# matthiasverstraete/3d_recognizer

Hardware: AMD Instinct MI355X
Metric: training clouds/sec, N=40960 pts, bs=8, at 1/2/4/8 GPUs; mIoU parity (higher is better)
Workload: dtype f32 storage/accumulate, bf16x3 MFMA in the wide GEMMs

## Files before the change

3d_recognizer_amd/csrc/bn.hip:

```cpp
#include "rl_common.h"

namespace {

__device__ __forceinline__ void slot_sums_wg(const double* __restrict__ stats, int nslots, int C, int c,
                                             double (*red)[2], double& s_out, double& q_out) {
    const int t = threadIdx.x;
    double s = 0.0, q = 0.0;
    const double* base = stats + c;
    for (int i = t; i < nslots; i += 256) {
        s += base[((long)i * 2 + 0) * C];
        q += base[((long)i * 2 + 1) * C];
    }
    s = rl_wave_sum(s);
    q = rl_wave_sum(q);
    if ((t & 63) == 0) { red[t >> 6][0] = s; red[t >> 6][1] = q; }
    __syncthreads();
    s_out = (red[0][0] + red[1][0]) + (red[2][0] + red[3][0]);
    q_out = (red[0][1] + red[1][1]) + (red[2][1] + red[3][1]);
}

__device__ __forceinline__ void slot_sums(const double* __restrict__ stats, int nslots, int C, int c, int lane,
                                          double& s_out, double& q_out) {
    double s0 = 0.0, s1 = 0.0, s2 = 0.0, s3 = 0.0, q0 = 0.0, q1 = 0.0, q2 = 0.0, q3 = 0.0;
    const double* base = stats + c;
// ... 195 lines not shown
                                                                   float* coef0, float* dgamma1, float* dbeta1, float* coef1) {
    __shared__ double red[4][2];
    if (blockIdx.y == 0) bn_bwd_finalize_body(stats0, nslots, count, C, dgamma0, dbeta0, coef0, (int)blockIdx.x, red);
    else bn_bwd_finalize_body(stats1, nslots, count, C, dgamma1, dbeta1, coef1, (int)blockIdx.x, red);
}

constexpr int BNBF_MAX = 8;
struct BnBwdFinBatch {
    rl_bn_bwd_finalize_item it[BNBF_MAX];
};
__global__ __launch_bounds__(256) void bn_bwd_finalize_batch_kernel(const BnBwdFinBatch b) {
    __shared__ double red[4][2];
    const rl_bn_bwd_finalize_item& t = b.it[blockIdx.y];
    if ((int)blockIdx.x >= t.C) return;
    bn_bwd_finalize_body(t.stats, t.nslots, (double)t.count, t.C, t.dgamma, t.dbeta, t.coef, (int)blockIdx.x, red);
}

__global__ __launch_bounds__(256) void bn_bwd_apply_kernel(const BwdParams p) {
    const int C = p.C;
    const int tpr = C < 256 ? C : 256;
    const int rpar = 256 / tpr;
    const int col = threadIdx.x % tpr, rsub = threadIdx.x / tpr;
    if (rsub >= rpar) return;
    const long ntiles = (p.M + p.tile - 1) / p.tile;
    for (long tile = blockIdx.x; tile < ntiles; tile += gridDim.x) {
        const long rend = min(p.M, (tile + 1) * p.tile);
        for (long R = tile * p.tile + rsub; R < rend; R += rpar) {
            const long off = row_off(p, R);
            for (int c = col; c < C; c += 256) {
                const float y = p.Y[off + c];
                const float sc = p.scale ? p.scale[c] : 1.f, sh = p.shift ? p.shift[c] : 0.f;
                float g = p.G[off + c] * rl_act_grad(y * sc + sh, p.act, p.slope);
                if (p.coef) {
                    const float xh = (y - p.mean[c]) * p.invstd[c];
                    g = g - p.coef[c] - xh * p.coef[C + c];
                }
                p.G[off + c] = sc * g;
            }
        }
    }
}

typedef float bnf4 __attribute__((ext_vector_type(4)));
struct BnQuad {
    bnf4 sc, sh, mu, is;
    float neg;
    __device__ __forceinline__ void load(const BwdParams& p, int c, bool want_xhat) {
        sc = p.scale ? *reinterpret_cast<const bnf4*>(p.scale + c) : (bnf4){1.f, 1.f, 1.f, 1.f};
        sh = p.shift ? *reinterpret_cast<const bnf4*>(p.shift + c) : (bnf4){0.f, 0.f, 0.f, 0.f};
        mu = (bnf4){0.f, 0.f, 0.f, 0.f};
        is = mu;
        if (want_xhat) {
            mu = *reinterpret_cast<const bnf4*>(p.mean + c);
            is = *reinterpret_cast<const bnf4*>(p.invstd + c);
        }
        neg = p.act == RL_ACT_RELU ? 0.f : (p.act == RL_ACT_LRELU ? p.slope : 1.f);
    }
    __device__ __forceinline__ bnf4 grad(const bnf4 y, const bnf4 gin) const {
        const bnf4 z = y * sc + sh;
        bnf4 d;
// ... 51 lines not shown
        for (int j = 0; j < 4; ++j) {
            p.stats[((long)blockIdx.x * 2 + 0) * C + c + j] = s[j];
            p.stats[((long)blockIdx.x * 2 + 1) * C + c + j] = s[4 + j];
        }
    }
}

__global__ __launch_bounds__(256) void bn_bwd_apply_vec_kernel(const BwdParams p) {
    const int C = p.C, c4 = C >> 2;
    const int tpr = c4 < 256 ? c4 : 256;
    const int rpar = 256 / tpr;
    const int q = threadIdx.x % tpr, rsub = threadIdx.x / tpr;
    const int c = q * 4;
    const bool full = p.coef != nullptr;
    BnQuad k;
    k.load(p, c, full);
    bnf4 k0 = {0.f, 0.f, 0.f, 0.f}, k1 = k0;
    if (full) {
        k0 = *reinterpret_cast<const bnf4*>(p.coef + c);
        k1 = *reinterpret_cast<const bnf4*>(p.coef + C + c);
    }
    const bnf4 osc = p.scale ? k.sc : (bnf4){1.f, 1.f, 1.f, 1.f};
    auto row = [&](const bnf4 y, const bnf4 gi) {
        bnf4 g = k.grad(y, gi);
        if (full) g = g - k0 - k.xhat(y) * k1;
        return g * osc;
    };
    const long ntiles = (p.M + p.tile - 1) / p.tile;
    for (long tile = blockIdx.x; tile < ntiles; tile += gridDim.x) {
        const long rend = min(p.M, (tile + 1) * p.tile);
        long R = tile * p.tile + rsub;
        for (; R + rpar < rend; R += 2 * rpar) {
            const long o0 = row_off(p, R) + c, o1 = row_off(p, R + rpar) + c;
            const bnf4 y0 = *reinterpret_cast<const bnf4*>(p.Y + o0), g0 = *reinterpret_cast<const bnf4*>(p.G + o0);
            const bnf4 y1 = *reinterpret_cast<const bnf4*>(p.Y + o1), g1 = *reinterpret_cast<const bnf4*>(p.G + o1);
            *reinterpret_cast<bnf4*>(p.G + o0) = row(y0, g0);
            *reinterpret_cast<bnf4*>(p.G + o1) = row(y1, g1);
        }
        if (R < rend) {
            const long o0 = row_off(p, R) + c;
            const bnf4 y0 = *reinterpret_cast<const bnf4*>(p.Y + o0), g0 = *reinterpret_cast<const bnf4*>(p.G + o0);
            *reinterpret_cast<bnf4*>(p.G + o0) = row(y0, g0);
        }
    }
}

struct ResidParams {
    float* G; float* G2; const float* O; float slope; long M; int C;
    const float* Y1; const float* sc1; const float* mu1; const float* is1;
// ... 445 lines not shown
```

3d_recognizer_amd/csrc/gemm.hip:

```cpp
#include "rl_common.h"
#include <stdlib.h>
#include <string.h>

namespace {

typedef float f32x4 __attribute__((ext_vector_type(4)));

constexpr int GM_BM = 128;
constexpr int GM_BK = 16;
constexpr int GM_AS = 20;

struct AOperand {
    const float* A;
    long lda, a_bstride;
    int a_mode;
    RlLazy lazy;
    const float* xyz;
    long xyz_bstride;
    const int32_t* nbr_idx;
    const float* nbr_d2;
    int nbr_k;
    int n;
    int K;
    long M;
// ... 750 lines not shown
template <int KT, int NT>
__global__ __launch_bounds__(256) void swgrad_kernel(const WgradParams p) {
    __shared__ float red[KT * NT * 4 * 64 + NT * 64];
    swgrad_body<KT, NT>(p, (int)blockIdx.x, red);
}

void swgrad_split(long M, int* nsplit, long* rows_per_block) {
    constexpr long rows_wg = 256;
    long want = (M + rows_wg - 1) / rows_wg;
    const long fill = (M + 127) / 128 < 256 ? (M + 127) / 128 : 256;
    if (want < fill) want = fill;
    if (want < 1) want = 1;
    if (want > 1024) want = 1024;
    long rpb = (M + want - 1) / want;
    rpb = ((rpb + 63) / 64) * 64;
    *rows_per_block = rpb;
    *nsplit = (int)((M + rpb - 1) / rpb);
    if (*nsplit < 1) *nsplit = 1;
}

inline bool stream_ok(int N, int K) { return (N <= 64 && K <= 64) || (K <= 16 && N <= 128); }

constexpr int swgrad_body_index(int KT, int NT) { return 4 * (KT >= 4 ? 2 : KT - 1) + (NT >= 8 ? 3 : NT >= 4 ? 2 : NT - 1); }

constexpr int PG_BK = 32;
constexpr int PG_AS = 36;

typedef __attribute__((ext_vector_type(8))) __bf16 bf16x8;
typedef __attribute__((ext_vector_type(4))) __bf16 bf16x4;

template <int NT, bool STATS>
__device__ __forceinline__ void tile_rows_epilogue(const GemmParams& p, const f32x4 (&acc)[NT], long Rb, int col0, int lr, int lq,
                                                   float (&ssum)[NT], float (&ssq)[NT]) {
    constexpr int BN = 16 * NT;
    const int N = p.N;
    const long M = p.a.M;
    const bool to_y = !p.out2 || col0 + BN <= p.split_col;
    const bool to_out2 = p.out2 && !p.out2_index && col0 >= p.split_col;
    if (to_y || to_out2) {
        const bool full = col0 + BN <= N;
        const bool has_bias = p.bias != nullptr;
        const bool accumulate = to_y && p.accumulate;
        float bv[NT];
#pragma unroll
        for (int nb = 0; nb < NT; ++nb) {
            const int c = col0 + nb * 16 + lr;
// ... 2126 lines not shown
extern "C" int rl_wgrad_reduce_batch(const rl_wgrad_reduce_item* items, int count, void* stream) {
    RL_REQUIRE(items != nullptr && count >= 0, RL_ERR_ARGS, "rl_wgrad_reduce_batch: bad arguments");
    hipStream_t st = (hipStream_t)stream;
    for (int base = 0; base < count; base += RB_MAX) {
        ReduceBatch b;
        b.count = count - base < RB_MAX ? count - base : RB_MAX;
        long tiles = 0;
        for (int i = 0; i < b.count; ++i) {
            const rl_wgrad_reduce_item& it = items[base + i];
            RL_REQUIRE(it.slab && it.dW && it.nsplit > 0 && it.N > 0 && it.K > 0, RL_ERR_ARGS,
                       "rl_wgrad_reduce_batch: bad item %d", base + i);
            b.item[i] = it;
            b.first_tile[i] = (int)tiles;
            tiles += rl_cdiv((long)it.N * it.K + it.N, WR_E);
            RL_REQUIRE(tiles < (1l << 30), RL_ERR_ARGS, "rl_wgrad_reduce_batch: too many tiles");
        }
        b.first_tile[b.count] = (int)tiles;
        hipLaunchKernelGGL(wgrad_reduce_batch_kernel, dim3((unsigned)tiles), dim3(256), 0, st, b);
        RL_LAUNCH_CHECK("rl_wgrad_reduce_batch");
    }
    rl_note_kernel("wgrad_reduce_batch_kernel");
    return RL_OK;
}
```

3d_recognizer_amd/csrc/rl_common.h:

```cpp
#pragma once
#include <hip/hip_runtime.h>
#include <stdarg.h>
#include <stdint.h>
#include <stdio.h>

#include "../../include/rl_randlanet.h"

void rl_set_error(const char* fmt, ...);
void rl_note_kernel(const char* name);

#define RL_REQUIRE(cond, code, ...)      \
    do {                                 \
        if (!(cond)) {                   \
            rl_set_error(__VA_ARGS__);   \
            return (code);               \
        }                                \
    } while (0)

#define RL_LAUNCH_CHECK(name)                                                        \
    do {                                                                             \
        hipError_t e_ = hipGetLastError();                                           \
        if (e_ != hipSuccess) {                                                      \
            rl_set_error("%s: launch failed: %s", name, hipGetErrorString(e_));      \
            return RL_ERR_LAUNCH;                                                    \
// ... 17 lines not shown
    const char* e = getenv("RL_ALLOW_FLOAT_ATOMICS");
    return e && e[0] == '1';
}

static inline int rl_row_blocks_host(long rows, int rows_per_tile) {
    long tiles = (rows + rows_per_tile - 1) / rows_per_tile;
    if (tiles < 1) tiles = 1;
    return (int)(tiles < RL_MAX_SLOTS ? tiles : RL_MAX_SLOTS);
}

#define RL_ACT_NONE 0
#define RL_ACT_RELU 1
#define RL_ACT_LRELU 2

__device__ __forceinline__ float rl_act(float z, int act, float slope) {
    if (act == RL_ACT_RELU) return z > 0.f ? z : 0.f;
    if (act == RL_ACT_LRELU) return z > 0.f ? z : z * slope;
    return z;
}
__device__ __forceinline__ float rl_act_grad(float z, int act, float slope) {
    if (act == RL_ACT_RELU) return z > 0.f ? 1.f : 0.f;
    if (act == RL_ACT_LRELU) return z > 0.f ? 1.f : slope;
    return 1.f;
}

struct RlLazy {
    const float* scale;
    const float* shift;
    int act;
    float slope;
};
__device__ __forceinline__ float rl_lazy(const RlLazy& t, float raw, int c) {
    if (t.scale == nullptr) return raw;
    return rl_act(raw * t.scale[c] + t.shift[c], t.act, t.slope);
}

typedef __bf16 rl_bf16x4 __attribute__((ext_vector_type(4)));
template <bool BF>
__device__ __forceinline__ float rl_ldx(const float* p, long i) {
    if constexpr (BF) return (float)reinterpret_cast<const __bf16*>(p)[i];
    else return p[i];
}
template <bool BF>
__device__ __forceinline__ void rl_stx(float* p, long i, float v) {
    if constexpr (BF) reinterpret_cast<__bf16*>(p)[i] = (__bf16)v;
    else p[i] = v;
// ... 55 lines not shown
```

3d_recognizer_amd/randlanet/_engine.py:

```python
from typing import Dict, List, Optional

import torch

from . import _hip as H
from . import _ops as ops
from ._ops import Lazy, Rpe

BN_EPS = 1e-6
BN_MOMENTUM = 0.99
BN_PIVOT = True
BAND_SORT_MIN_POINTS = 4096


class _Tape(list):

    def __init__(self):
        super().__init__()
        self.levels: List[int] = []

    def append(self, rec) -> None:
        super().append(rec)
        self.levels.append(ops.LEVEL)

    def clear(self) -> None:
# ... 458 lines not shown
                ops.scale_mask(G, mask, scale)
                ctx.grads[id(src.raw)] = [G, True]
            else:
                raise AssertionError(kind)
        self._flush_rpe(ctx)
        ops.LEVEL = -1
        ops.wgrad_batch_flush(ctx.wbatch)
        ops.wgrad_flush(ctx.pending)
        ctx.tape.clear()
        ctx.grads.clear()
        ctx.keep.clear()

    def _flush_rpe(self, ctx: Context) -> None:
        if ctx.fin_queue:
            first = ctx.fin_queue.pop(0)
            ops._bn_bwd_finalize(*first, None, also=ctx.fin_queue)
        for fn in ctx.rpe_after:
            fn()
        ctx.rpe_after.clear()

    def _bwd_linear(self, ctx, grads, a, out: Lazy, wname, bname, ks, ns, a_grad):
        G, init = self._gbuf(ctx, out)
        assert init, f"no gradient reached {wname}"
        if out.scale is not None and id(out.raw) not in ctx.bn_done:
            ops.bn_backward(G, out, grads[f"{out.bn}.weight"], grads[f"{out.bn}.bias"], True, sync=self.sync,
                            stats=ctx.bn_pre.pop(id(out.raw), None), also=ctx.fin_queue)
            self._flush_rpe(ctx)
        n_out = out.C
        ops.wgrad(a, G, out.bstride, n_out, grads[wname], ks, ns, grads[bname] if bname else None, pending=ctx.pending,
                  batch=ctx.wbatch)
        halves = getattr(a, "concat", None) if (a_grad and isinstance(a, Lazy)) else None
        if (halves is not None and (n_out > 64 or a.C > 64) and id(a.raw) not in ctx.grads
                and halves[1].bstride == halves[1].n and halves[1].raw.shape[0] == a.rows
                and halves[1].raw.shape[1] == halves[1].C and halves[0].C % 4 == 0
                and not ctx.grads.get(id(halves[1].raw), (None, False))[1]):
            prev, skip = halves
            gs = self._gbuf(ctx, skip)
            Gp = torch.empty((a.rows, prev.C), dtype=torch.float32, device=G.device)
            gl = Lazy(G, out.B, out.n, out.bstride, n_out)
            ops.gemm(gl, self._w2(wname), ns, ks, a.C, None, out=Gp, out_bstride=a.bstride, out2=gs[0], split_col=prev.C,
                     wsplit=getattr(ctx, "wsplit", None))
            gs[1] = True
            ctx.grads[id(a.raw)] = [Gp, "split"]
            return
        if a_grad and isinstance(a, Lazy):
            ga = self._gbuf(ctx, a)
            if not ga[1]:
                assert a.n == a.bstride and a.raw.shape[0] == a.B * a.n, "first writer must cover the tensor"
            gl = Lazy(G, out.B, out.n, out.bstride, n_out)
            complete = (self.sync is None and a.scale is not None and a.mean is not None and a.rows == a.raw.shape[0] and
                        ((not ga[1] and (wname in ("fc_end.1.conv.weight", "fc_end.0.conv.weight") or wname.endswith(".mlp2.conv.weight")))
                         or (ga[1] and wname == "encoder.0.mlp1.conv.weight")))
            res = ops.gemm(gl, self._w2(wname), ns, ks, a.C, None, out=ga[0], out_bstride=a.bstride, accumulate=ga[1],
                           wsplit=getattr(ctx, "wsplit", None), bnb=a if complete else None)
            if complete and res[1] is not None:
                ctx.bn_pre[id(a.raw)] = res[1]
            ga[1] = True

    def _bwd_pool_virtual(self, ctx, grads, name, vr, g: Lazy, csr, idx, pooled: Lazy, n, d, stage):
        h = d // 2
        e = name.rsplit(".", 1)[0]
        GP, init = self._gbuf(ctx, pooled)
        assert init
        key = ("vgu", id(vr))
        if stage == 2:
            GU = torch.empty((vr.rows, h), dtype=ops.row_dtype(), device=GP.device)
            first = True
        else:
            GU, first = ctx.grads.pop(key)[0], False
        gg = self._gbuf(ctx, g)
        nslots = H.lib().rl_pool_bwd_slots(vr.B * n, d)
        bstats = torch.empty((nslots, 2, h), dtype=torch.float64, device=GP.device)
        DG = ops.pool_bwd(vr, g, idx, self.P[f"{name}.score_fn.0.weight"], n, d, GP, GU, not first,
                          grads[f"{name}.score_fn.0.weight"], pending=ctx.pending, stage=stage, bn_bwd_stats=bstats)
        ops.segment_sum_rows(DG, (0, h), n * self.K, csr, gg[0], g.bstride, accumulate=gg[1])
        gg[1] = True
        layer = f"{e}.mlp_rpe{stage}"
        queue = ctx.fin_queue if self.sync is None else None
        coef = ops.rpe_bn_backward(vr, stage, GU, grads[f"{layer}.batch_norm.weight"], grads[f"{layer}.batch_norm.bias"],
                                   sync=self.sync, stats=bstats, nslots=nslots, queue=queue)
# ... 37 lines not shown
```

3d_recognizer_amd/randlanet/_hip.py:

```python
import ctypes as C
import os
from typing import Optional

import torch

_LIB: Optional[C.CDLL] = None
_LIB_PATH = os.path.join(os.path.dirname(os.path.dirname(os.path.abspath(__file__))), "csrc",
                         "librandla_hip.so")
_LIB_PATH = os.environ.get("RL_HIP_LIB", _LIB_PATH)

ABI_VERSION = 110
MAX_SLOTS = 1024
KNN_MAX_K = 64
ACT_NONE, ACT_RELU, ACT_LRELU = 0, 1, 2

ERR_ARGS, ERR_FEW_SUPPORT, ERR_LAUNCH, ERR_UNSUPPORTED = -1, -2, -3, -4


class HipKernelError(RuntimeError):
    pass


class GemmDesc(C.Structure):
    _fields_ = [
# ... 195 lines not shown
    "rl_get_wide_gemm": (C.c_char_p, []),
    "rl_set_wgemm_staging": (_i, [C.c_char_p]),
    "rl_set_wgemm_tile": (_i, [C.c_char_p]),
    "rl_set_gemm_ksplit": (_i, [_i]),
    "rl_set_sgemm_grid_div": (_i, [_i]),
    "rl_wgrad": (_i, [C.POINTER(WgradDesc), _vp]),
    "rl_wgrad_nsplit": (_i, [_l, _i, _i]),
    "rl_wgrad_batchable": (_i, [C.POINTER(WgradDesc)]),
    "rl_wgrad_batch": (_i, [C.POINTER(WgradDesc), _i, _vp]),
    "rl_wgrad_reduce_batch": (_i, [C.POINTER(WgradReduceItem), _i, _vp]),
    "rl_bn_finalize": (_i, [_vp, _i, _l, _i, _vp, _vp, _vp, _vp, _vp, _f, _f, _i, _vp, _vp, _vp, _vp, _vp, _i, _vp, _vp]),
    "rl_bn_finalize_batch": (_i, [C.POINTER(BnFinalizeItem), _i, _vp]),
    "rl_bn_bwd_finalize_batch": (_i, [C.POINTER(BnBwdFinalizeItem), _i, _vp]),
    "rl_head_supported": (_i, [_i, _i]),
    "rl_head_grid": (_i, [_l]),
    "rl_head_fwd": (_i, [C.POINTER(HeadDesc), _vp, _vp]),
    "rl_head_bwd": (_i, [C.POINTER(HeadDesc), _vp]),
    "rl_bn_bwd_finalize_pair": (_i, [_vp, _vp, _i, _l, _i, _vp, _vp, _vp, _vp, _vp, _vp, _vp]),
    "rl_bn_reduce_slots": (_i, [_vp, _i, _i, _vp, _vp]),
    "rl_bn_bwd_slots": (_i, [_l]),
    "rl_bn_bwd_reduce": (_i, [C.POINTER(BnBwdDesc), _vp]),
    "rl_bn_bwd_finalize": (_i, [_vp, _i, _l, _i, _vp, _vp, _vp, _vp]),
    "rl_bn_bwd_apply": (_i, [C.POINTER(BnBwdDesc), _vp]),
    "rl_bn_bwd_fused_supported": (_i, [_l, _i, _l]),
    "rl_bn_bwd_fused": (_i, [C.POINTER(BnBwdDesc), _l, _vp, _vp, _vp, _vp]),
    "rl_resid_bn_bwd_supported": (_i, [_l, _i]),
    "rl_resid_bn_bwd_reduce": (_i, [C.POINTER(ResidBnBwdDesc), _vp]),
    "rl_resid_bn_bwd_apply": (_i, [C.POINTER(ResidBnBwdDesc), _vp]),
    "rl_resid_bn_bwd_fused_supported": (_i, [_l, _i]),
    "rl_resid_bn_bwd_fused": (_i, [C.POINTER(ResidBnBwdDesc), _vp, _vp, _vp, _vp, _vp]),
    "rl_copy_rows": (_i, [C.POINTER(RowsDesc), _vp]),
    "rl_copy_rows_pair": (_i, [C.POINTER(RowsDesc), C.POINTER(RowsDesc), _vp]),
    "rl_scatter_add_rows": (_i, [C.POINTER(RowsDesc), _vp]),
    "rl_csr_workspace_bytes": (_l, [C.POINTER(CsrTask), _i, _i]),
    "rl_csr_build": (_i, [C.POINTER(CsrTask), _i, _i, _vp, _l, _vp]),
    "rl_segment_sum_rows": (_i, [C.POINTER(SegsumDesc), _vp]),
    "rl_pool_supported": (_i, [_i, _i]),
    "rl_pool_slab_floats": (_l, [_l, _i]),
    "rl_pool_bwd_slots": (_i, [_l, _i]),
    "rl_pool_bwd_grid": (_i, [_l, _i, _i]),
    "rl_pool_fwd_slots": (_i, [_l, _i]),
    "rl_pool_fwd": (_i, [C.POINTER(PoolDesc), _vp]),
    "rl_rpe_stats_slots": (_i, [_l]),
    "rl_rpe_stats": (_i, [C.POINTER(PoolDesc), _vp, _vp]),
    "rl_rpe_bn_reduce": (_i, [C.POINTER(PoolDesc), _vp, _vp, _vp]),
    "rl_rpe_wgrad_slab_floats": (_l, [_l, _i, _i]),
# ... 96 lines not shown
```

3d_recognizer_amd/randlanet/_ops.py:

```python
import ctypes as C
import os
from dataclasses import dataclass
from typing import Optional, Tuple

import torch

from . import _hip as H

F32 = torch.float32
BF16 = torch.bfloat16

_STORAGE = os.environ.get("RL_STORAGE", "f32")


def set_storage(mode: str) -> None:
    global _STORAGE
    if mode not in ("f32", "bf16"):
        raise ValueError(f"storage must be 'f32' or 'bf16', got {mode!r}")
    if mode == "bf16" and get_wide_gemm() == "fp32":
        raise H.HipKernelError("bf16 storage needs the bf16x3 / bf16 arithmetic mode (RL_WIDE_GEMM)")
    _STORAGE = mode


def get_storage() -> str:
# ... 582 lines not shown
        _bn_bwd_finalize(stats[0], stats[1], y.rows, y.C, dgamma, dbeta, coef, None, also=also)
        d.coef = coef.data_ptr()
        with _rec("bn_bwd_apply", (y.rows, y.C), 12 * y.rows * y.C, 0):
            H.check(H.lib().rl_bn_bwd_apply(C.byref(d), _st()), "rl_bn_bwd_apply")
        return not also
    if (training and y.mean is not None and sync is None and not NO_BN_SMALL and G.data_ptr() % 16 == 0 and y.raw.data_ptr() % 16 == 0
            and H.lib().rl_bn_bwd_fused_supported(y.rows, y.C, y.raw.shape[1])):
        with _rec("bn_bwd_fused", (y.rows, y.C), 12 * y.rows * y.C, 0):
            H.check(H.lib().rl_bn_bwd_fused(C.byref(d), y.rows, H.ptr(dgamma), H.ptr(dbeta), None, _st()), "rl_bn_bwd_fused")
        return not also
    if training and y.mean is not None:
        stats = new_stats(G.device, y.C)
        coef = torch.empty(2 * y.C, dtype=F32, device=G.device)
        d.stats = stats.data_ptr()
        with _rec("bn_bwd_reduce", (y.rows, y.C), 8 * y.rows * y.C, 0):
            H.check(H.lib().rl_bn_bwd_reduce(C.byref(d), _st()), "rl_bn_bwd_reduce")
        _bn_bwd_finalize(stats, H.lib().rl_bn_bwd_slots(y.rows), y.rows, y.C, dgamma, dbeta, coef, sync, also=also)
        d.coef = coef.data_ptr()
    with _rec("bn_bwd_apply", (y.rows, y.C), 12 * y.rows * y.C, 0):
        H.check(H.lib().rl_bn_bwd_apply(C.byref(d), _st()), "rl_bn_bwd_apply")
    return not also


def resid_bn_supported(y1: Lazy, y2: Lazy) -> bool:
    dense = all(y.bstride == y.n and y.raw.shape == (y.B * y.n, y.C) and y.mean is not None and y.act == H.ACT_NONE for y in (y1, y2))
    return dense and y1.C == y2.C and y1.rows == y2.rows and bool(H.lib().rl_resid_bn_bwd_supported(y1.rows, y1.C))


def resid_bn_backward(G: torch.Tensor, O: torch.Tensor, slope: float, y1: Lazy, y2: Lazy, dgamma1, dbeta1, dgamma2, dbeta2,
                      sync: Optional[SyncGroup] = None):
    _dev_check(G, O, y1.raw, y2.raw)
    rows, Cc = y1.rows, y1.C
    assert G.shape == O.shape == (rows, Cc)
    d = H.ResidBnBwdDesc()
    G2 = torch.empty_like(G)
    d.G, d.G2, d.O, d.slope, d.rows, d.C = G.data_ptr(), G2.data_ptr(), O.data_ptr(), slope, rows, Cc
    d.Y1, d.scale1, d.mean1, d.invstd1 = y1.raw.data_ptr(), y1.scale.data_ptr(), y1.mean.data_ptr(), y1.invstd.data_ptr()
    d.Y2, d.scale2, d.mean2, d.invstd2 = y2.raw.data_ptr(), y2.scale.data_ptr(), y2.mean.data_ptr(), y2.invstd.data_ptr()
    if sync is None and not NO_BN_SMALL and H.lib().rl_resid_bn_bwd_fused_supported(rows, Cc):
        with _rec("resid_bn_bwd_fused", (rows, Cc), 24 * rows * Cc, 0):
            H.check(H.lib().rl_resid_bn_bwd_fused(C.byref(d), H.ptr(dgamma1), H.ptr(dbeta1), H.ptr(dgamma2), H.ptr(dbeta2), _st()),
                    "rl_resid_bn_bwd_fused")
        return G2
    st1, st2 = new_stats(G.device, Cc), new_stats(G.device, Cc)
    c1 = torch.empty(2 * Cc, dtype=F32, device=G.device)
    c2 = torch.empty(2 * Cc, dtype=F32, device=G.device)
# ... 659 lines not shown
```

include/rl_randlanet.h:

```cpp
#ifndef RL_RANDLANET_H
#define RL_RANDLANET_H

#include <stdint.h>

#ifdef __cplusplus
extern "C" {
#endif

#define RL_VERSION 110

#define RL_OK 0
#define RL_ERR_ARGS (-1)
#define RL_ERR_FEW_SUPPORT (-2)
#define RL_ERR_LAUNCH (-3)
#define RL_ERR_UNSUPPORTED (-4)

#define RL_MAX_SLOTS 1024
#define RL_KNN_MAX_K 64

const char* rl_last_error(void);
const char* rl_last_kernel(void);
int rl_version(void);
int64_t rl_launch_count(void);
int rl_spin_us(int us, void* stream);
// ... 169 lines not shown
    const float* mean;
    const float* invstd;
    double* stats;
    const float* coef;
} rl_bn_bwd_desc;

int rl_bn_reduce_slots(const double* stats, int nslots, int C, double* out, void* stream);
int rl_bn_bwd_slots(int64_t rows);
int rl_bn_bwd_reduce(const rl_bn_bwd_desc* d, void* stream);
int rl_bn_bwd_finalize(const double* stats, int nslots, int64_t count, int C, float* dgamma,
                       float* dbeta, float* coef, void* stream);
int rl_bn_bwd_finalize_pair(const double* stats0, const double* stats1, int nslots, int64_t count, int C, float* dgamma0,
                            float* dbeta0, float* coef0, float* dgamma1, float* dbeta1, float* coef1, void* stream);
typedef struct rl_bn_bwd_finalize_item {
    const double* stats;
    int64_t count;
    float* dgamma;
    float* dbeta;
    float* coef;
    int32_t nslots, C;
} rl_bn_bwd_finalize_item;
int rl_bn_bwd_finalize_batch(const rl_bn_bwd_finalize_item* items, int count, void* stream);
int rl_bn_bwd_apply(const rl_bn_bwd_desc* d, void* stream);
int rl_bn_bwd_fused_supported(int64_t rows, int C, int64_t ld);
int rl_bn_bwd_fused(const rl_bn_bwd_desc* d, int64_t count, float* dgamma, float* dbeta, float* coef_out, void* stream);

typedef struct rl_resid_bn_bwd_desc {
    float* G;
    float* G2;
    const float* O;
    float slope;
    int64_t rows;
    int32_t C;
    const float* Y1; const float* scale1; const float* mean1; const float* invstd1;
    const float* Y2; const float* scale2; const float* mean2; const float* invstd2;
    double* stats1; double* stats2;
    const float* coef1; const float* coef2;
} rl_resid_bn_bwd_desc;

int rl_resid_bn_bwd_supported(int64_t rows, int C);
int rl_resid_bn_bwd_reduce(const rl_resid_bn_bwd_desc* d, void* stream);
int rl_resid_bn_bwd_apply(const rl_resid_bn_bwd_desc* d, void* stream);
int rl_resid_bn_bwd_fused_supported(int64_t rows, int C);
int rl_resid_bn_bwd_fused(const rl_resid_bn_bwd_desc* d, float* dgamma1, float* dbeta1, float* dgamma2, float* dbeta2, void* stream);

typedef struct rl_rows_desc {
// ... 249 lines not shown
```

Measured before the change: 1286.

## Fuse BN backward apply, weight-grad and input-grad GEMMs into one linear-backward kernel

Adds a single streaming kernel for small linear layers (K,N ≤ 64) that applies the batch-norm backward elementwise transform, accumulates the weight and bias gradient into per-block slabs, and computes the input gradient with MFMA in one pass. It can also fold the next layer's BN backward statistics into the same epilogue. This removes separate bn_bwd_apply, wgrad and dgrad launches and the round trips of the intermediate gradient through global memory. The BN elementwise math is factored into a shared helper used by the existing apply kernels. The trade-off is heavy register and shared-memory use per block, plus a more complex planning and fallback path on the Python side.

```diff
diff --git a/3d_recognizer_amd/csrc/bn.hip b/3d_recognizer_amd/csrc/bn.hip
--- a/3d_recognizer_amd/csrc/bn.hip
+++ b/3d_recognizer_amd/csrc/bn.hip
@@ -241,20 +241,17 @@
     const int rpar = 256 / tpr;
     const int col = threadIdx.x % tpr, rsub = threadIdx.x / tpr;
     if (rsub >= rpar) return;
+    const float neg = p.act == RL_ACT_RELU ? 0.f : (p.act == RL_ACT_LRELU ? p.slope : 1.f);
     const long ntiles = (p.M + p.tile - 1) / p.tile;
     for (long tile = blockIdx.x; tile < ntiles; tile += gridDim.x) {
         const long rend = min(p.M, (tile + 1) * p.tile);
         for (long R = tile * p.tile + rsub; R < rend; R += rpar) {
             const long off = row_off(p, R);
             for (int c = col; c < C; c += 256) {
-                const float y = p.Y[off + c];
                 const float sc = p.scale ? p.scale[c] : 1.f, sh = p.shift ? p.shift[c] : 0.f;
-                float g = p.G[off + c] * rl_act_grad(y * sc + sh, p.act, p.slope);
-                if (p.coef) {
-                    const float xh = (y - p.mean[c]) * p.invstd[c];
-                    g = g - p.coef[c] - xh * p.coef[C + c];
-                }
-                p.G[off + c] = sc * g;
+                const bool full = p.coef != nullptr;
+                p.G[off + c] = rl_bn_bwd_elem(p.G[off + c], p.Y[off + c], sc, sh, full ? p.mean[c] : 0.f, full ? p.invstd[c] : 0.f,
+                                              full ? p.coef[c] : 0.f, full ? p.coef[C + c] : 0.f, neg, sc, full);
             }
         }
     }
@@ -352,9 +349,10 @@
     }
     const bnf4 osc = p.scale ? k.sc : (bnf4){1.f, 1.f, 1.f, 1.f};
     auto row = [&](const bnf4 y, const bnf4 gi) {
-        bnf4 g = k.grad(y, gi);
-        if (full) g = g - k0 - k.xhat(y) * k1;
-        return g * osc;
+        bnf4 g;
+#pragma unroll
+        for (int j = 0; j < 4; ++j) g[j] = rl_bn_bwd_elem(gi[j], y[j], k.sc[j], k.sh[j], k.mu[j], k.is[j], k0[j], k1[j], k.neg, osc[j], full);
+        return g;
     };
     const long ntiles = (p.M + p.tile - 1) / p.tile;
     for (long tile = blockIdx.x; tile < ntiles; tile += gridDim.x) {
diff --git a/3d_recognizer_amd/csrc/gemm.hip b/3d_recognizer_amd/csrc/gemm.hip
--- a/3d_recognizer_amd/csrc/gemm.hip
+++ b/3d_recognizer_amd/csrc/gemm.hip
@@ -796,6 +796,318 @@
 inline bool stream_ok(int N, int K) { return (N <= 64 && K <= 64) || (K <= 16 && N <= 128); }
 
 constexpr int swgrad_body_index(int KT, int NT) { return 4 * (KT >= 4 ? 2 : KT - 1) + (NT >= 8 ? 3 : NT >= 4 ? 2 : NT - 1); }
+
+struct LinBwdParams {
+    GemmParams g;
+    const float* Yl;
+    const float* sc; const float* sh; const float* mu; const float* is; const float* coef;
+    float neg;
+    AOperand in;
+    float* slab;
+    int has_bias;
+};
+
+constexpr int LB_TS = 68;
+
+template <int GC, int AT, bool DG, bool BNB>
+__global__ __launch_bounds__(256) void linbwd_kernel(const LinBwdParams p) {
+    __shared__ double sred[BNB ? 4 : 1][2][16 * AT];
+    __shared__ __attribute__((aligned(16))) float cf[6][16 * GC];
+    __shared__ __attribute__((aligned(16))) float tr[4][16 * LB_TS];
+    __shared__ float wred[GC * AT * 4 * 64 + GC * 64];
+    const int tid = threadIdx.x, lane = tid & 63, wave = __builtin_amdgcn_readfirstlane(tid >> 6);
+    const int li = lane & 15, lj = lane >> 4;
+    const GemmParams& g = p.g;
+    const AOperand& in = p.in;
+    const int C = g.a.K, Kin = in.K;
+    const long M = g.a.M;
+
+    for (int c = tid; c < 16 * GC; c += 256) {
+        const bool v = c < C;
+        cf[0][c] = v ? p.sc[c] : 1.f;   cf[1][c] = v ? p.sh[c] : 0.f;
+        cf[2][c] = v ? p.mu[c] : 0.f;   cf[3][c] = v ? p.is[c] : 0.f;
+        cf[4][c] = v ? p.coef[c] : 0.f; cf[5][c] = v ? p.coef[C + c] : 0.f;
+    }
+    __syncthreads();
+
+    float wf[DG ? GC : 1][4][DG ? AT : 1];
+    float bias[AT], ssum[AT], ssq[AT];
+    float bsc[BNB ? AT : 1], bsh[BNB ? AT : 1], bmu[BNB ? AT : 1], bis[BNB ? AT : 1];
+    if constexpr (DG) {
+#pragma unroll
+        for (int c = 0; c < GC; ++c)
+#pragma unroll
+            for (int s = 0; s < 4; ++s) {
+                const int k = 16 * c + 4 * lj + s;
+#pragma unroll
+                for (int t = 0; t < AT; ++t) {
+                    const int n = t * 16 + li;
+                    wf[c][s][t] = (k < C && n < g.N) ? g.W[(long)k * g.w_ks + (long)n * g.w_ns] : 0.f;
+                }
+            }
+    }
+#pragma unroll
+    for (int t = 0; t < AT; ++t) {
+        const int n = t * 16 + li;
+        bias[t] = (DG && g.bias && n < g.N) ? g.bias[n] : 0.f;
+        ssum[t] = ssq[t] = 0.f;
+        if constexpr (BNB) {
+            bsc[t] = n < g.N ? g.bnb_scale[n] : 1.f; bsh[t] = n < g.N ? g.bnb_shift[n] : 0.f;
+            bmu[t] = n < g.N ? g.bnb_mean[n] : 0.f;  bis[t] = n < g.N ? g.bnb_invstd[n] : 0.f;
+        }
+    }
+    const bool full = g.N == 16 * AT;
+    float isc[AT], ish[AT];
+#pragma unroll
+    for (int t = 0; t < AT; ++t) {
+        const int k = t * 16 + li;
+        isc[t] = (in.lazy.scale && k < Kin) ? in.lazy.scale[k] : 1.f;
+        ish[t] = (in.lazy.scale && k < Kin) ? in.lazy.shift[k] : 0.f;
+    }
+    const bool lazy = in.a_mode != 1 && in.lazy.scale != nullptr;
+    const float es = (!lazy || in.lazy.act == RL_ACT_NONE) ? 1.f : (in.lazy.act == RL_ACT_RELU ? 0.f : in.lazy.slope);
+
+    f32x4 accw[GC][AT];
+    float bsum[GC];
+#pragma unroll
+    for (int c = 0; c < GC; ++c) {
+        bsum[c] = 0.f;
+#pragma unroll
+        for (int t = 0; t < AT; ++t) accw[c][t] = (f32x4){0.f, 0.f, 0.f, 0.f};
+    }
+
+    const long nblk = (M + 15) >> 4;
+    const long bstep = (long)gridDim.x * 4;
+    auto fetch = [&](long blk, float4 (&gq)[GC], float4 (&yq)[GC], float (&av)[4][AT]) {
+        const long row = blk * 16 + li;
+        const bool rvalid = row < M;
+        const long goff = rvalid ? a_row_offset(g.a, row) : 0;
+#pragma unroll
+        for (int c = 0; c < GC; ++c) {
+            gq[c] = make_float4(0.f, 0.f, 0.f, 0.f);
+            yq[c] = gq[c];
+            if (rvalid && 16 * c + 4 * lj < C) {
+                gq[c] = *reinterpret_cast<const float4*>(g.a.A + goff + 16 * c + 4 * lj);
+                yq[c] = *reinterpret_cast<const float4*>(p.Yl + goff + 16 * c + 4 * lj);
+            }
+        }
+#pragma unroll
+        for (int r = 0; r < 4; ++r) {
+            const long R = blk * 16 + lj * 4 + r;
+            const bool valid = R < M;
+            if (in.a_mode == 1) {
+                float v = 0.f;
+                if (valid && li < 10) {
+                    if (li == 9) v = __fsqrt_rn(in.nbr_d2[R]);
+                    else {
+                        const long pt = (unsigned)R / (unsigned)in.nbr_k;
+                        const int b = (int)((unsigned)pt / (unsigned)in.n);
+                        const int i = (int)(pt - (long)b * in.n);
+                        const int ax = li % 3;
+                        const float* xb = in.xyz + (long)b * in.xyz_bstride * 3;
+                        const float xi = xb[(long)i * 3 + ax];
+                        if (li < 3) v = xi;
+                        else {
+                            const float xj = xb[(long)in.nbr_idx[R] * 3 + ax];
+                            v = li < 6 ? xj : xi - xj;
+                        }
+                    }
+                }
+                av[r][0] = v;
+#pragma unroll
+                for (int t = 1; t < AT; ++t) av[r][t] = 0.f;
+            } else {
+                const long ioff = valid ? a_row_offset(in, R) : 0;
+#pragma unroll
+                for (int t = 0; t < AT; ++t) {
+                    const int k = t * 16 + li;
+                    av[r][t] = (valid && k < Kin) ? in.A[ioff + k] : 0.f;
+                }
+            }
+        }
+    };
+
+    float4 gq[GC], yq[GC], gqn[GC], yqn[GC];
+    float av[4][AT], avn[4][AT];
+    float* const trw = tr[wave];
+    {
+        long blk = (long)blockIdx.x * 4 + wave;
+        if (blk < nblk) fetch(blk, gq, yq, av);
+        for (; blk < nblk; blk += bstep) {
+            const bool rvalid = blk * 16 + li < M;
+            if (blk + bstep < nblk) fetch(blk + bstep, gqn, yqn, avn);
+            float dr[GC][4];
+#pragma unroll
+            for (int c = 0; c < GC; ++c) {
+                const int col = 16 * c + 4 * lj;
+                const float4 s4 = *reinterpret_cast<const float4*>(&cf[0][col]), h4 = *reinterpret_cast<const float4*>(&cf[1][col]);
+                const float4 m4 = *reinterpret_cast<const float4*>(&cf[2][col]), i4 = *reinterpret_cast<const float4*>(&cf[3][col]);
+                const float4 k04 = *reinterpret_cast<const float4*>(&cf[4][col]), k14 = *reinterpret_cast<const float4*>(&cf[5][col]);
+                const bool ok = rvalid && col < C;
+                dr[c][0] = ok ? rl_bn_bwd_elem(gq[c].x, yq[c].x, s4.x, h4.x, m4.x, i4.x, k04.x, k14.x, p.neg, s4.x, true) : 0.f;
+                dr[c][1] = ok ? rl_bn_bwd_elem(gq[c].y, yq[c].y, s4.y, h4.y, m4.y, i4.y, k04.y, k14.y, p.neg, s4.y, true) : 0.f;
+                dr[c][2] = ok ? rl_bn_bwd_elem(gq[c].z, yq[c].z, s4.z, h4.z, m4.z, i4.z, k04.z, k14.z, p.neg, s4.z, true) : 0.f;
+                dr[c][3] = ok ? rl_bn_bwd_elem(gq[c].w, yq[c].w, s4.w, h4.w, m4.w, i4.w, k04.w, k14.w, p.neg, s4.w, true) : 0.f;
+                *reinterpret_cast<float4*>(trw + li * LB_TS + col) = make_float4(dr[c][0], dr[c][1], dr[c][2], dr[c][3]);
+            }
+            f32x4 acc[AT];
+            if constexpr (DG) {
+#pragma unroll
+                for (int t = 0; t < AT; ++t) acc[t] = (f32x4){0.f, 0.f, 0.f, 0.f};
+#pragma unroll
+                for (int c = 0; c < GC; ++c)
+#pragma unroll
+                    for (int s = 0; s < 4; ++s)
+#pragma unroll
+                        for (int t = 0; t < AT; ++t)
+                            acc[t] = __builtin_amdgcn_mfma_f32_16x16x4f32(dr[c][s], wf[c][s][t], acc[t], 0, 0, 0);
+            }
+            __builtin_amdgcn_fence(__ATOMIC_RELEASE, "wavefront");
+            __builtin_amdgcn_wave_barrier();
+            __builtin_amdgcn_fence(__ATOMIC_ACQUIRE, "wavefront");
+#pragma unroll
+            for (int r = 0; r < 4; ++r) {
+                const bool valid = blk * 16 + lj * 4 + r < M;
+                float ap[AT];
+#pragma unroll
+                for (int t = 0; t < AT; ++t) {
+                    float v = av[r][t];
+                    if (lazy) {
+                        const float z = v * isc[t] + ish[t];
+                        v = fmaxf(z, z * es);
+                    }
+                    ap[t] = (valid && t * 16 + li < Kin) ? v : 0.f;
+                }
+#pragma unroll
+                for (int c = 0; c < GC; ++c) {
+                    const float dt = trw[(lj * 4 + r) * LB_TS + 16 * c + li];
+                    bsum[c] += dt;
+#pragma unroll
+                    for (int t = 0; t < AT; ++t) accw[c][t] = __builtin_amdgcn_mfma_f32_16x16x4f32(dt, ap[t], accw[c][t], 0, 0, 0);
+                }
+            }
+            __builtin_amdgcn_fence(__ATOMIC_RELEASE, "wavefront");
+            __builtin_amdgcn_wave_barrier();
+            if constexpr (DG) {
+                asm volatile("" ::: "memory");
+                __builtin_amdgcn_s_waitcnt(0x0F70);
+                asm volatile("" ::: "memory");
+#pragma unroll
+                for (int r = 0; r < 4; ++r) {
+                    const long R = blk * 16 + lj * 4 + r;
+                    if (R < M) {
+                        long yoff;
+                        if (g.y_contig) yoff = R * g.ldy;
+                        else {
+                            const int b = (int)((unsigned)R / (unsigned)g.rows_per_batch);
+                            const int i = (int)(R - (long)b * g.rows_per_batch);
+                            yoff = ((long)b * g.y_bstride + i) * g.ldy;
+                        }
+                        float* y = g.Y + yoff + li;
+                        float v[AT];
+#pragma unroll
+                        for (int t = 0; t < AT; ++t) v[t] = acc[t][r] + bias[t];
+                        if (g.accumulate) {
+                            float o[AT];
+#pragma unroll
+                            for (int t = 0; t < AT; ++t) o[t] = (full || t * 16 + li < g.N) ? y[t * 16] : 0.f;
+#pragma unroll
+                            for (int t = 0; t < AT; ++t) v[t] += o[t];
+                        }
+#pragma unroll
+                        for (int t = 0; t < AT; ++t) {
+                            if (full || t * 16 + li < g.N) {
+                                y[t * 16] = v[t];
+                                if constexpr (BNB) {
+                                    const float tv = av[r][t];
+                                    const float z = tv * bsc[t] + bsh[t];
+                                    const float gp = v[t] * (z > 0.f ? 1.f : g.bnb_neg);
+                                    ssum[t] += gp;
+                                    ssq[t] += gp * ((tv - bmu[t]) * bis[t]);
+                                }
+                            }
+                        }
+                    }
+                }
+            }
+#pragma unroll
+            for (int c = 0; c < GC; ++c) { gq[c] = gqn[c]; yq[c] = yqn[c]; }
+#pragma unroll
+            for (int r = 0; r < 4; ++r)
+#pragma unroll
+                for (int t = 0; t < AT; ++t) av[r][t] = avn[r][t];
+        }
+        if constexpr (BNB) {
+#pragma unroll
+            for (int t = 0; t < AT; ++t) {
+                float s = ssum[t], q = ssq[t];
+                s += __shfl_xor(s, 16, 64); s += __shfl_xor(s, 32, 64);
+                q += __shfl_xor(q, 16, 64); q += __shfl_xor(q, 32, 64);
+                if (lane < 16) {
+                    sred[wave][0][t * 16 + lane] = (double)s;
+                    sred[wave][1][t * 16 + lane] = (double)q;
+                }
+            }
+            __syncthreads();
+            const int N = g.N;
+            if (tid < 16 * AT && tid < N) {
+                g.stats[((long)blockIdx.x * 2 + 0) * N + tid] = sred[0][0][tid] + sred[1][0][tid] + sred[2][0][tid] + sred[3][0][tid];
+                g.stats[((long)blockIdx.x * 2 + 1) * N + tid] = sred[0][1][tid] + sred[1][1][tid] + sred[2][1][tid] + sred[3][1][tid];
+                for (long slot = blockIdx.x + gridDim.x; slot < g.stat_slots; slot += gridDim.x) {
+                    g.stats[(slot * 2 + 0) * N + tid] = 0.0;
+                    g.stats[(slot * 2 + 1) * N + tid] = 0.0;
+                }
+            }
+        }
+    }
+#pragma unroll
+    for (int c = 0; c < GC; ++c) {
+        bsum[c] += __shfl_xor(bsum[c], 16, 64);
+        bsum[c] += __shfl_xor(bsum[c], 32, 64);
+    }
+    float* rb = wred + GC * AT * 4 * 64;
+    for (int w = 1; w < 4; ++w) {
+        __syncthreads();
+        if (wave == w) {
+#pragma unroll
+            for (int c = 0; c < GC; ++c) {
+#pragma unroll
+                for (int t = 0; t < AT; ++t)
+#pragma unroll
+                    for (int r = 0; r < 4; ++r) wred[((c * AT + t) * 4 + r) * 64 + lane] = accw[c][t][r];
+                rb[c * 64 + lane] = bsum[c];
+            }
+        }
+        __syncthreads();
+        if (wave == 0) {
+#pragma unroll
+            for (int c = 0; c < GC; ++c) {
+#pragma unroll
+                for (int t = 0; t < AT; ++t)
+#pragma unroll
+                    for (int r = 0; r < 4; ++r) accw[c][t][r] += wred[((c * AT + t) * 4 + r) * 64 + lane];
+                bsum[c] += rb[c * 64 + lane];
+            }
+        }
+    }
+    if (wave == 0) {
+        float* out = p.slab + (long)blockIdx.x * ((long)C * Kin + C);
+#pragma unroll
+        for (int c = 0; c < GC; ++c) {
+#pragma unroll
+            for (int t = 0; t < AT; ++t) {
+                const int k = t * 16 + li;
+#pragma unroll
+                for (int r = 0; r < 4; ++r) {
+                    const int n = c * 16 + lj * 4 + r;
+                    if (n < C && k < Kin) out[(long)n * Kin + k] = accw[c][t][r];
+                }
+            }
+            const int n = c * 16 + li;
+            if (p.has_bias && lj == 0 && n < C) out[(long)C * Kin + n] = bsum[c];
+        }
+    }
+}
 
 constexpr int PG_BK = 32;
 constexpr int PG_AS = 36;
@@ -2968,3 +3280,103 @@
     rl_note_kernel("wgrad_reduce_batch_kernel");
     return RL_OK;
 }
+
+namespace {
+
+typedef void (*LinBwdFn)(const LinBwdParams);
+struct LinBwdPlan {
+    LinBwdFn fn;
+    int nsplit;
+    const char* refusal;
+};
+
+template <int GC, int AT>
+LinBwdFn linbwd_inst(bool dg, bool bnb) {
+    return !dg ? linbwd_kernel<GC, AT, false, false> : bnb ? linbwd_kernel<GC, AT, true, true> : linbwd_kernel<GC, AT, true, false>;
+}
+template <int GC>
+LinBwdFn linbwd_fn(int Kin, bool dg, bool bnb) {
+    return Kin <= 16 ? linbwd_inst<GC, 1>(dg, bnb) : Kin <= 32 ? linbwd_inst<GC, 2>(dg, bnb) : linbwd_inst<GC, 4>(dg, bnb);
+}
+
+LinBwdPlan plan_linear_bwd(long M, int C, int Kin, bool dg, bool bnb) {
+    LinBwdPlan pl{};
+    if (C > 64 || Kin > 64 || C % 4) { pl.refusal = "rl_linear_bwd: the streaming class only (K <= 64, N <= 64, N % 4 == 0)"; return pl; }
+    const GemmPlan gp = plan_gemm(GemmFacts{M, Kin, C, true, false, false, false, false, false, dg && bnb, 0});
+    if (gp.kernel != GK_SGEMM) { pl.refusal = "rl_linear_bwd: the input-gradient product is not the streaming kernel's"; return pl; }
+    pl.nsplit = (int)gp.grid.x;
+    pl.fn = C <= 16 ? linbwd_fn<1>(Kin, dg, bnb) : C <= 32 ? linbwd_fn<2>(Kin, dg, bnb) : linbwd_fn<4>(Kin, dg, bnb);
+    return pl;
+}
+
+int linbwd_fill(const rl_gemm_desc* dg, const rl_bn_bwd_desc* bn, const rl_wgrad_desc* wg, LinBwdParams* pp, LinBwdPlan* plan) {
+    const char* who = "rl_linear_bwd";
+    RL_REQUIRE(bn != nullptr && wg != nullptr, RL_ERR_ARGS, "%s: null descriptor", who);
+    LinBwdParams& p = *pp;
+    RL_REQUIRE(bn->G && bn->Y && bn->scale && bn->shift && bn->mean && bn->invstd, RL_ERR_UNSUPPORTED,
+               "%s: needs a BatchNorm layer in training mode (scale / shift / mean / invstd)", who);
+    RL_REQUIRE(bn->C > 0 && bn->C % 4 == 0 && bn->ld % 4 == 0 && ((((uintptr_t)bn->G) | ((uintptr_t)bn->Y)) & 15) == 0, RL_ERR_UNSUPPORTED,
+               "%s: G / Y rows must be 16-byte aligned with C %% 4 == 0", who);
+    int rc = fill_a(&p.g.a, who, bn->G, bn->ld, bn->bstride, 0, 0, 0.f, nullptr, nullptr, nullptr, 0, nullptr, nullptr, 0, bn->B, bn->n, bn->C);
+    if (rc) return rc;
+    p.Yl = bn->Y; p.sc = bn->scale; p.sh = bn->shift; p.mu = bn->mean; p.is = bn->invstd; p.coef = bn->coef;
+    p.neg = bn->act == RL_ACT_RELU ? 0.f : (bn->act == RL_ACT_LRELU ? bn->slope : 1.f);
+    RL_REQUIRE(!wg->rows_bf16 && wg->N == bn->C && wg->dY == bn->G && wg->lddy == bn->ld && wg->dy_bstride == bn->bstride, RL_ERR_UNSUPPORTED,
+               "%s: the weight gradient must read G (fp32 rows, the BatchNorm descriptor's layout)", who);
+    rc = fill_a(&p.in, who, wg->A, wg->lda, wg->a_bstride, wg->a_mode, wg->in_act, wg->in_slope, wg->in_scale, wg->in_shift,
+                wg->xyz, wg->xyz_bstride, wg->nbr_idx, wg->nbr_d2, wg->nbr_k, wg->B, wg->n, wg->K);
+    if (rc) return rc;
+    const int rows_per_batch = wg->a_mode == 1 ? wg->n * wg->nbr_k : wg->n;
+    RL_REQUIRE(p.in.M == p.g.a.M && wg->B == bn->B && rows_per_batch == bn->n, RL_ERR_UNSUPPORTED, "%s: A and G differ in their rows", who);
+    p.has_bias = wg->dbias != nullptr;
+    p.slab = wg->slab;
+    bool bnb = false;
+    if (dg) {
+        RL_REQUIRE(wg->a_mode == 0 && dg->a_mode == 0 && dg->A == bn->G && dg->lda == bn->ld && dg->a_bstride == bn->bstride && dg->B == bn->B &&
+                   dg->n == bn->n && dg->K == bn->C && dg->N == wg->K && !dg->in_scale, RL_ERR_UNSUPPORTED,
+                   "%s: the input-gradient product must read G as a plain tensor and have the input's columns", who);
+        RL_REQUIRE(dg->W && dg->Y && dg->ldy >= dg->N && dg->y_bstride >= dg->n && !dg->addend && !dg->out2, RL_ERR_UNSUPPORTED, "%s: bad W / dA", who);
+        bnb = dg->bnb_Y != nullptr;
+        RL_REQUIRE(bnb || !dg->stats, RL_ERR_UNSUPPORTED, "%s: forward statistics are not a by-product of this launch", who);
+        p.g.N = dg->N; p.g.W = dg->W; p.g.w_ks = dg->w_ks; p.g.w_ns = dg->w_ns; p.g.bias = dg->bias;
+        p.g.Y = dg->Y; p.g.ldy = dg->ldy; p.g.y_bstride = dg->y_bstride; p.g.rows_per_batch = dg->n;
+        p.g.y_contig = (dg->y_bstride == dg->n);
+        p.g.accumulate = dg->accumulate;
+        if (bnb) {
+            RL_REQUIRE(dg->bnb_Y == wg->A && dg->ldy == wg->lda && dg->y_bstride == wg->a_bstride, RL_ERR_UNSUPPORTED,
+                       "%s: bnb_Y must be the layer's input tensor, in dA's layout", who);
+            RL_REQUIRE(dg->stats && dg->bnb_scale && dg->bnb_shift && dg->bnb_mean && dg->bnb_invstd && !dg->stats_pivot_mean, RL_ERR_ARGS,
+                       "%s: bnb_Y needs stats, the layer's scale / shift / mean / invstd and no pivot", who);
+            p.g.stats = dg->stats;
+            p.g.bnb_Y = dg->bnb_Y; p.g.bnb_scale = dg->bnb_scale; p.g.bnb_shift = dg->bnb_shift; p.g.bnb_mean = dg->bnb_mean; p.g.bnb_invstd = dg->bnb_invstd;
+            p.g.bnb_neg = dg->bnb_act == RL_ACT_RELU ? 0.f : (dg->bnb_act == RL_ACT_LRELU ? dg->bnb_slope : 1.f);
+            p.g.stat_slots = (int)rl_gemm_stat_slots(p.g.a.M, dg->N, dg->K);
+        }
+    }
+    const LinBwdPlan pl = plan_linear_bwd(p.g.a.M, bn->C, wg->K, dg != nullptr, bnb);
+    RL_REQUIRE(pl.fn != nullptr, RL_ERR_UNSUPPORTED, "%s", pl.refusal);
+    *plan = pl;
+    return RL_OK;
+}
+
+}
+
+extern "C" int rl_linear_bwd_supported(const rl_gemm_desc* dgrad, const rl_bn_bwd_desc* bn, const rl_wgrad_desc* wg) {
+    LinBwdParams p{};
+    LinBwdPlan pl;
+    return linbwd_fill(dgrad, bn, wg, &p, &pl) == RL_OK ? pl.nsplit : 0;
+}
+
+extern "C" int rl_linear_bwd(const rl_gemm_desc* dgrad, const rl_bn_bwd_desc* bn, const rl_wgrad_desc* wg, void* stream) {
+    LinBwdParams p{};
+    LinBwdPlan pl;
+    int rc = linbwd_fill(dgrad, bn, wg, &p, &pl);
+    if (rc) return rc;
+    RL_REQUIRE(bn->coef != nullptr, RL_ERR_ARGS, "rl_linear_bwd: needs the means of rl_bn_bwd_finalize (coef)");
+    RL_REQUIRE(wg->slab && wg->defer_reduce && wg->slab_floats >= (int64_t)pl.nsplit * ((int64_t)wg->N * wg->K + wg->N), RL_ERR_ARGS,
+               "rl_linear_bwd: needs a private slab of rl_linear_bwd_supported() x (N*K + N) floats (defer_reduce set)");
+    hipLaunchKernelGGL(pl.fn, dim3(pl.nsplit), dim3(256), 0, (hipStream_t)stream, p);
+    rl_note_kernel("linbwd_kernel");
+    RL_LAUNCH_CHECK("rl_linear_bwd");
+    return RL_OK;
+}
diff --git a/3d_recognizer_amd/csrc/rl_common.h b/3d_recognizer_amd/csrc/rl_common.h
--- a/3d_recognizer_amd/csrc/rl_common.h
+++ b/3d_recognizer_amd/csrc/rl_common.h
@@ -63,6 +63,14 @@
     if (act == RL_ACT_RELU) return z > 0.f ? 1.f : 0.f;
     if (act == RL_ACT_LRELU) return z > 0.f ? 1.f : slope;
     return 1.f;
+}
+
+__device__ __forceinline__ float rl_bn_bwd_elem(float g, float y, float sc, float sh, float mu, float is, float k0, float k1,
+                                                float neg, float osc, bool full) {
+    const float z = __fadd_rn(__fmul_rn(y, sc), sh);
+    float d = __fmul_rn(g, z > 0.f ? 1.f : neg);
+    if (full) d = __fsub_rn(__fsub_rn(d, k0), __fmul_rn(__fmul_rn(__fsub_rn(y, mu), is), k1));
+    return __fmul_rn(d, osc);
 }
 
 struct RlLazy {
diff --git a/3d_recognizer_amd/randlanet/_engine.py b/3d_recognizer_amd/randlanet/_engine.py
--- a/3d_recognizer_amd/randlanet/_engine.py
+++ b/3d_recognizer_amd/randlanet/_engine.py
@@ -504,18 +504,21 @@
     def _bwd_linear(self, ctx, grads, a, out: Lazy, wname, bname, ks, ns, a_grad):
         G, init = self._gbuf(ctx, out)
         assert init, f"no gradient reached {wname}"
+        n_out = out.C
+        halves = getattr(a, "concat", None) if (a_grad and isinstance(a, Lazy)) else None
+        split = (halves is not None and (n_out > 64 or a.C > 64) and id(a.raw) not in ctx.grads
+                 and halves[1].bstride == halves[1].n and halves[1].raw.shape[0] == a.rows
+                 and halves[1].raw.shape[1] == halves[1].C and halves[0].C % 4 == 0
+                 and not ctx.grads.get(id(halves[1].raw), (None, False))[1])
         if out.scale is not None and id(out.raw) not in ctx.bn_done:
+            if self.sync is None and not split and n_out <= 64 and self._bwd_linear_fused(ctx, grads, a, out, G, wname, bname, ks, ns, a_grad):
+                return
             ops.bn_backward(G, out, grads[f"{out.bn}.weight"], grads[f"{out.bn}.bias"], True, sync=self.sync,
                             stats=ctx.bn_pre.pop(id(out.raw), None), also=ctx.fin_queue)
             self._flush_rpe(ctx)
-        n_out = out.C
         ops.wgrad(a, G, out.bstride, n_out, grads[wname], ks, ns, grads[bname] if bname else None, pending=ctx.pending,
                   batch=ctx.wbatch)
-        halves = getattr(a, "concat", None) if (a_grad and isinstance(a, Lazy)) else None
-        if (halves is not None and (n_out > 64 or a.C > 64) and id(a.raw) not in ctx.grads
-                and halves[1].bstride == halves[1].n and halves[1].raw.shape[0] == a.rows
-                and halves[1].raw.shape[1] == halves[1].C and halves[0].C % 4 == 0
-                and not ctx.grads.get(id(halves[1].raw), (None, False))[1]):
+        if split:
             prev, skip = halves
             gs = self._gbuf(ctx, skip)
             Gp = torch.empty((a.rows, prev.C), dtype=torch.float32, device=G.device)
@@ -530,14 +533,40 @@
             if not ga[1]:
                 assert a.n == a.bstride and a.raw.shape[0] == a.B * a.n, "first writer must cover the tensor"
             gl = Lazy(G, out.B, out.n, out.bstride, n_out)
-            complete = (self.sync is None and a.scale is not None and a.mean is not None and a.rows == a.raw.shape[0] and
-                        ((not ga[1] and (wname in ("fc_end.1.conv.weight", "fc_end.0.conv.weight") or wname.endswith(".mlp2.conv.weight")))
-                         or (ga[1] and wname == "encoder.0.mlp1.conv.weight")))
+            complete = self._completes(a, ga, wname)
             res = ops.gemm(gl, self._w2(wname), ns, ks, a.C, None, out=ga[0], out_bstride=a.bstride, accumulate=ga[1],
                            wsplit=getattr(ctx, "wsplit", None), bnb=a if complete else None)
             if complete and res[1] is not None:
                 ctx.bn_pre[id(a.raw)] = res[1]
             ga[1] = True
+
+    def _completes(self, a: Lazy, ga, wname) -> bool:
+        return (self.sync is None and a.scale is not None and a.mean is not None and a.rows == a.raw.shape[0] and
+                ((not ga[1] and (wname in ("fc_end.1.conv.weight", "fc_end.0.conv.weight") or wname.endswith(".mlp2.conv.weight")))
+                 or (ga[1] and wname == "encoder.0.mlp1.conv.weight")))
+
+    def _bwd_linear_fused(self, ctx, grads, a, out: Lazy, G, wname, bname, ks, ns, a_grad) -> bool:
+        if not isinstance(a, (Lazy, ops.Rpe)) or (isinstance(a, Lazy) and a.C > 64):
+            return False
+        ga = self._gbuf(ctx, a) if (a_grad and isinstance(a, Lazy)) else None
+        if ga is not None and not ga[1]:
+            assert a.n == a.bstride and a.raw.shape[0] == a.B * a.n, "first writer must cover the tensor"
+        complete = ga is not None and self._completes(a, ga, wname)
+        key = id(out.raw)
+        res = ops.linear_bwd(a, G, out, self._w2(wname), ns, ks, grads[wname], ks, ns, grads[bname] if bname else None,
+                             grads[f"{out.bn}.weight"], grads[f"{out.bn}.bias"], ctx.pending,
+                             stats=ctx.bn_pre.get(key), also=ctx.fin_queue,
+                             dA=ga[0] if ga is not None else None, dA_bstride=a.bstride if ga is not None else None,
+                             accumulate=bool(ga[1]) if ga is not None else False, bnb=a if complete else None)
+        if res is None:
+            return False
+        ctx.bn_pre.pop(key, None)
+        self._flush_rpe(ctx)
+        if ga is not None:
+            if res[1] is not None:
+                ctx.bn_pre[id(a.raw)] = res[1]
+            ga[1] = True
+        return True
 
     def _bwd_pool_virtual(self, ctx, grads, name, vr, g: Lazy, csr, idx, pooled: Lazy, n, d, stage):
         h = d // 2
diff --git a/3d_recognizer_amd/randlanet/_hip.py b/3d_recognizer_amd/randlanet/_hip.py
--- a/3d_recognizer_amd/randlanet/_hip.py
+++ b/3d_recognizer_amd/randlanet/_hip.py
@@ -241,6 +241,8 @@
     "rl_bn_bwd_reduce": (_i, [C.POINTER(BnBwdDesc), _vp]),
     "rl_bn_bwd_finalize": (_i, [_vp, _i, _l, _i, _vp, _vp, _vp, _vp]),
     "rl_bn_bwd_apply": (_i, [C.POINTER(BnBwdDesc), _vp]),
+    "rl_linear_bwd_supported": (_i, [C.POINTER(GemmDesc), C.POINTER(BnBwdDesc), C.POINTER(WgradDesc)]),
+    "rl_linear_bwd": (_i, [C.POINTER(GemmDesc), C.POINTER(BnBwdDesc), C.POINTER(WgradDesc), _vp]),
     "rl_bn_bwd_fused_supported": (_i, [_l, _i, _l]),
     "rl_bn_bwd_fused": (_i, [C.POINTER(BnBwdDesc), _l, _vp, _vp, _vp, _vp]),
     "rl_resid_bn_bwd_supported": (_i, [_l, _i]),
diff --git a/3d_recognizer_amd/randlanet/_ops.py b/3d_recognizer_amd/randlanet/_ops.py
--- a/3d_recognizer_amd/randlanet/_ops.py
+++ b/3d_recognizer_amd/randlanet/_ops.py
@@ -628,6 +628,70 @@
     return not also
 
 
+NO_LINEAR_BWD = False
+
+
+def linear_bwd(a, G: torch.Tensor, y: Lazy, W: torch.Tensor, dg_ks: int, dg_ns: int, dW: torch.Tensor, w_ks: int, w_ns: int,
+               dbias: Optional[torch.Tensor], dgamma: torch.Tensor, dbeta: torch.Tensor, pending: list, *,
+               stats: Optional[tuple] = None, also: Optional[list] = None, dA: Optional[torch.Tensor] = None,
+               dA_bstride: Optional[int] = None, accumulate: bool = False, bnb: Optional[Lazy] = None):
+    if NO_LINEAR_BWD or pending is None or y.scale is None or y.mean is None or G.dtype != F32 or y.raw.dtype != F32:
+        return None
+    if not isinstance(a, Rpe) and a.raw.dtype != F32:
+        return None
+    if (stats is None and not NO_BN_SMALL and G.data_ptr() % 16 == 0 and y.raw.data_ptr() % 16 == 0
+            and H.lib().rl_bn_bwd_fused_supported(y.rows, y.C, y.raw.shape[1])):
+        return None
+    N = y.C
+    bn = _bn_bwd_desc(G, y.bstride, y)
+    wg = H.WgradDesc()
+    M, K = _fill_a(wg, a)
+    _dev_check(dW, dbias, W, dA)
+    assert dW.numel() == K * N and (dbias is None or dbias.numel() == N) and W.numel() == K * N
+    wg.N, wg.dY, wg.lddy, wg.dy_bstride = N, G.data_ptr(), G.shape[1], y.bstride
+    wg.dW, wg.w_ks, wg.w_ns, wg.dbias, wg.defer_reduce = dW.data_ptr(), w_ks, w_ns, H.ptr(dbias), 1
+    dg = bnb_pre = None
+    if dA is not None:
+        assert not isinstance(a, Rpe) and dA.dtype == F32 and dA.dim() == 2 and dA.shape[1] >= K
+        dA_bstride = a.n if dA_bstride is None else dA_bstride
+        assert dA.shape[0] >= (a.B - 1) * dA_bstride + a.n, "dA rows out of range"
+        dg = H.GemmDesc()
+        _fill_a(dg, Lazy(G, y.B, y.n, y.bstride, N))
+        dg.N, dg.W, dg.w_ks, dg.w_ns = K, W.data_ptr(), dg_ks, dg_ns
+        dg.Y, dg.ldy, dg.y_bstride, dg.accumulate = dA.data_ptr(), dA.shape[1], dA_bstride, int(accumulate)
+        if (bnb is not None and bnb.raw is a.raw and bnb.mean is not None and bnb.scale is not None
+                and bnb.raw.shape[1] == dA.shape[1] and bnb.bstride == dA_bstride and bnb.C == K):
+            _dev_check(bnb.raw, bnb.scale, bnb.shift, bnb.mean, bnb.invstd)
+            st_b = new_stats(W.device, K)
+            dg.stats = st_b.data_ptr()
+            dg.bnb_Y, dg.bnb_scale, dg.bnb_shift = bnb.raw.data_ptr(), bnb.scale.data_ptr(), bnb.shift.data_ptr()
+            dg.bnb_mean, dg.bnb_invstd, dg.bnb_act, dg.bnb_slope = bnb.mean.data_ptr(), bnb.invstd.data_ptr(), bnb.act, bnb.slope
+            bnb_pre = (st_b, gemm_stat_slots(M, K, N))
+    nsplit = H.lib().rl_linear_bwd_supported(C.byref(dg) if dg is not None else None, C.byref(bn), C.byref(wg))
+    if nsplit <= 0:
+        return None
+    coef = torch.empty(2 * N, dtype=F32, device=G.device)
+    if stats is None:
+        st = new_stats(G.device, N)
+        bn.stats = st.data_ptr()
+        with _rec("bn_bwd_reduce", (y.rows, N), 8 * y.rows * N, 0):
+            H.check(H.lib().rl_bn_bwd_reduce(C.byref(bn), _st()), "rl_bn_bwd_reduce")
+        stats = (st, H.lib().rl_bn_bwd_slots(y.rows))
+    _bn_bwd_finalize(stats[0], stats[1], y.rows, N, dgamma, dbeta, coef, None, also=also)
+    bn.coef = coef.data_ptr()
+    slab = torch.empty(nsplit * (N * K + N), dtype=F32, device=G.device)
+    wg.slab, wg.slab_floats = slab.data_ptr(), slab.numel()
+    k_in = 6 if isinstance(a, Rpe) else K
+    nbytes = 4 * M * (2 * N + k_in + (K * (2 if accumulate else 1) if dg is not None else 0))
+    with _rec("linear_bwd", (M, K, N), nbytes, (4 if dg is not None else 2) * M * K * N):
+        H.check(H.lib().rl_linear_bwd(C.byref(dg) if dg is not None else None, C.byref(bn), C.byref(wg), _st()), "rl_linear_bwd")
+    it = H.WgradReduceItem()
+    it.slab, it.dW, it.dbias, it.w_ks, it.w_ns = slab.data_ptr(), dW.data_ptr(), H.ptr(dbias), w_ks, w_ns
+    it.nsplit, it.N, it.K = nsplit, N, K
+    pending.append((it, slab, dW, dbias))
+    return True, bnb_pre
+
+
 def resid_bn_supported(y1: Lazy, y2: Lazy) -> bool:
     dense = all(y.bstride == y.n and y.raw.shape == (y.B * y.n, y.C) and y.mean is not None and y.act == H.ACT_NONE for y in (y1, y2))
     return dense and y1.C == y2.C and y1.rows == y2.rows and bool(H.lib().rl_resid_bn_bwd_supported(y1.rows, y1.C))
diff --git a/include/rl_randlanet.h b/include/rl_randlanet.h
--- a/include/rl_randlanet.h
+++ b/include/rl_randlanet.h
@@ -215,6 +215,9 @@
 } rl_bn_bwd_finalize_item;
 int rl_bn_bwd_finalize_batch(const rl_bn_bwd_finalize_item* items, int count, void* stream);
 int rl_bn_bwd_apply(const rl_bn_bwd_desc* d, void* stream);
+
+int rl_linear_bwd_supported(const rl_gemm_desc* dgrad, const rl_bn_bwd_desc* bn, const rl_wgrad_desc* wg);
+int rl_linear_bwd(const rl_gemm_desc* dgrad, const rl_bn_bwd_desc* bn, const rl_wgrad_desc* wg, void* stream);
 int rl_bn_bwd_fused_supported(int64_t rows, int C, int64_t ld);
 int rl_bn_bwd_fused(const rl_bn_bwd_desc* d, int64_t count, float* dgamma, float* dbeta, float* coef_out, void* stream);
 
```

Result: slower. 1270 (-1.2%).
